# ogulcanaydogan/llm-slo-ebpf-toolkit

Measured on AMD Instinct MI355X. Metric: fault-replay attribution throughput through the agent's BPF-ring -> GPU path (events/s, node-wide); held-out attribution macro-F1 and agent CPU overhead % reported alongside, higher is better.
Workload: dtype fp64 posteriors / fp32 features (exact-int64 time joins)

## Files before the change

### llm_slo_ebpf_toolkit_amd/ops/csrc/agent_bindings.cpp

```cpp
#include <pybind11/numpy.h>
#include <pybind11/pybind11.h>
#include <pybind11/stl.h>

#include <cstring>
#include <memory>
#include <stdexcept>

#include "decodesli.h"
#include "drift.h"
#include "engine.h"
#include "errsli.h"
#include "exemplars.h"
#include "onset.h"
#include "openreq.h"
#include "podrank.h"
#include "slisketch.h"

namespace py = pybind11;
using namespace mislo;

namespace {

template <class T>
py::array_t<T> copy_array(const T* p, std::vector<py::ssize_t> shape) {
// ... 1222 lines not shown
      .def("resident", &PyErrorSliTracker::resident)
      .def("sync", &PyErrorSliTracker::sync)
      .def("close", &PyErrorSliTracker::close);
  py::class_<PyEngine>(m, "WindowEngine")
      .def(py::init<int, int, int, int, int, int, int, double, double, int, int, bool, bool, int, float, double, int,
                    int, int, int, int, bool>(),
           py::arg("device") = 0, py::arg("sig_cap") = 1 << 20, py::arg("span_cap") = 16384, py::arg("group_cap") = 64,
           py::arg("user_cap") = 1 << 18, py::arg("n_buffers") = 3, py::arg("max_ahead") = 3,
           py::arg("window_ms") = 2000.0, py::arg("threshold") = 0.7, py::arg("fanout") = 3, py::arg("group_mode") = 1,
           py::arg("use_graphs") = true, py::arg("device_refit") = true, py::arg("n_dom") = 10,
           py::arg("ttft_slo_ms") = 800.0f, py::arg("halo_ms") = 0.0, py::arg("import_cap") = 0,
           py::arg("xchg_cap") = 0, py::arg("shard_rank") = 0, py::arg("shard_world") = 1,
           py::arg("halo_windows") = 3, py::arg("split_rings") = false)
      .def("register_host", &PyEngine::register_host)
      .def("submit", &PyEngine::submit, py::arg("k"), py::arg("kernel"), py::arg("user"), py::arg("spans"),
           py::arg("n_groups"), py::arg("labels") = py::none(), py::arg("bases") = std::vector<int64_t>{},
           py::arg("with_labels") = true, py::arg("learn") = false, py::arg("user_rec") = 64)
      .def("submit_copy", &PyEngine::submit_copy, py::arg("k"), py::arg("kernel"), py::arg("user"), py::arg("spans"),
           py::arg("n_groups"), py::arg("labels") = py::none(), py::arg("bases") = std::vector<int64_t>{},
           py::arg("user_rec") = 64)
      .def("submit_chain", &PyEngine::submit_chain, py::arg("k"), py::arg("n_groups"), py::arg("with_labels") = true,
           py::arg("learn") = false)
      .def("h2d_done", &PyEngine::h2d_done)
      .def("wait_h2d", &PyEngine::wait_h2d)
      .def("query", &PyEngine::query)
      .def("wait", &PyEngine::wait)
      .def("packet", &PyEngine::packet)
      .def("results", &PyEngine::results)
      .def("window_ms", &PyEngine::window_ms)
      .def("copy_ms", [](PyEngine& p, int64_t k) {
        py::gil_scoped_release nogil;
        return p.eng().copy_ms(k);
      })
      .def("set_model_bytes", &PyEngine::set_model_bytes)
      .def("set_app_model", &PyEngine::set_app_model)
      .def("set_p0", &PyEngine::set_p0)
      .def("set_refit", &PyEngine::set_refit, py::arg("alpha") = 2.0, py::arg("prior_pseudo") = 1.0,
           py::arg("inv_temp") = 1.0, py::arg("min_count") = 0.0, py::arg("cap_dom") = -1, py::arg("ceil") = 1.0)
      .def("refit_now", &PyEngine::refit_now)
      .def("set_device_refit", [](PyEngine& p, bool on) { p.eng().set_device_refit(on); })
      .def("score", &PyEngine::score, py::arg("feat"), py::arg("labels") = py::none(), py::arg("app") = py::none())
      .def("set_pods", &PyEngine::set_pods)
      .def("inject_remote", &PyEngine::inject_remote)
      .def("results_all", &PyEngine::results_all)
      .def("set_join_params", &PyEngine::set_join_params)
      .def("init_comm", &PyEngine::init_comm)
      .def("totals", &PyEngine::totals)
      .def("reset_totals", &PyEngine::reset_totals)
      .def("stats_acc", &PyEngine::stats_acc)
      .def("model_bytes", &PyEngine::model_bytes)
      .def("restore", &PyEngine::restore)
      .def("sync", &PyEngine::sync)
      .def("import_state", &PyEngine::import_state)
      .def("sent_block", &PyEngine::sent_block)
      .def("close", &PyEngine::close)
      .def_property_readonly("buffers", &PyEngine::buffers)
      .def_property_readonly("copy_lanes", [](PyEngine& p) { return p.eng().copy_lanes(); })
      .def_property_readonly("copy_ahead", [](PyEngine& p) { return p.eng().copy_ahead(); })
      .def("take_copy_lanes", [](PyEngine& p) {
        py::gil_scoped_release nogil;
        return p.eng().take_copy_lanes();
      })
      .def_property_readonly("windows_folded", &PyEngine::folded)
      .def_property_readonly("graphs", &PyEngine::graphs)
      .def_property_readonly("host_issue_us", &PyEngine::host_issue_us)
      .def_property_readonly("host_wait_us", &PyEngine::host_wait_us)
// ... 12 lines not shown
```

### llm_slo_ebpf_toolkit_amd/ops/csrc/decode.hip

```cpp
#include "mislo_common.h"
#include "mislo_launch.h"
#include <stdexcept>

namespace mislo {

__constant__ Tables c_tab;

struct DecodeOut {
  SignalCols cols;
  uint32_t* hist;
  uint32_t* status_cnt;
  uint32_t* part_cnt;
  unsigned long long* misc;
  int blk_base = 0;
  uint32_t* sel_cnt = nullptr;
  unsigned long long* sel_mask = nullptr;
  int sel_stride = 0;
};

constexpr int kMiscSums = 2;

template <int NT>
__device__ __forceinline__ void store_counts(const uint32_t* lds, uint32_t* dst) {
  for (int i = threadIdx.x; i < kKeyTypes * kParts; i += NT) dst[i] = lds[i];
}

struct DecodeLds {
  alignas(16) Tables tab;
  static constexpr int kRep = 8, kPartRep = 4;
  static constexpr int kHS = kSlots * kBuckets + 1, kSS = kSlots * 3 + 1, kUS = kSlots + 1;
  static constexpr int kPS = kKeyTypes * kParts + 1;
  uint32_t hist[kRep * kHS];
  uint32_t status[kRep * kSS];
  uint32_t part[kPartRep * kPS];
  unsigned long long sum[kRep * kUS];
};

template <int NT>
__device__ __forceinline__ void lds_init(DecodeLds& L) {
  static_assert(sizeof(Tables) % 4 == 0 && offsetof(Tables, edges) % 16 == 0, "table layout");
  {
    const uint32_t* src = reinterpret_cast<const uint32_t*>(&c_tab);
    uint32_t* dst = reinterpret_cast<uint32_t*>(&L.tab);
    for (int i = threadIdx.x; i < (int)(sizeof(Tables) / 4); i += NT) dst[i] = src[i];
  }
  for (int i = threadIdx.x; i < DecodeLds::kPartRep * DecodeLds::kPS; i += NT) L.part[i] = 0;
  for (int i = threadIdx.x; i < DecodeLds::kRep * DecodeLds::kUS; i += NT) L.sum[i] = 0;
  for (int i = threadIdx.x; i < DecodeLds::kRep * DecodeLds::kHS; i += NT) L.hist[i] = 0;
  for (int i = threadIdx.x; i < DecodeLds::kRep * DecodeLds::kSS; i += NT) L.status[i] = 0;
  __syncthreads();
}

struct LdsLane {
  uint32_t *hist, *status, *part;
  unsigned long long* sum;
  const Tables* tab;
};
__device__ __forceinline__ LdsLane lds_lane(DecodeLds& L) {
  const int r = threadIdx.x & (DecodeLds::kRep - 1), q = threadIdx.x & (DecodeLds::kPartRep - 1);
  return LdsLane{L.hist + r * DecodeLds::kHS, L.status + r * DecodeLds::kSS, L.part + q * DecodeLds::kPS,
                 L.sum + r * DecodeLds::kUS, &L.tab};
}
// ... 585 lines not shown
    }
    PartCodes pc;
#pragma unroll
    for (int k = 0; k < kKeyTypes; ++k) {
      const uint64_t h = r.ts != 0 ? key_hash(k, r.tr, r.pod, r.pid, r.cn, r.sn) : 0ull;
      pc.p[k] = h ? (uint16_t)part_of(h) : kNoPart;
      if (h) atomicAdd(&s_part[k * kParts + part_of(h)], 1u);
    }
    c.part[i] = pc;
  }
  if (sm.gen) {
    for (int off = 32; off > 0; off >>= 1) {
      t_lo = min(t_lo, (uint64_t)__shfl_xor((long long)t_lo, off));
      t_hi = max(t_hi, (uint64_t)__shfl_xor((long long)t_hi, off));
    }
    if ((threadIdx.x & 63) == 0 && t_lo <= t_hi) {
      atomicMin(reinterpret_cast<unsigned long long*>(&sm.gen->span_lo), (unsigned long long)t_lo);
      atomicMax(reinterpret_cast<unsigned long long*>(&sm.gen->span_hi), (unsigned long long)t_hi);
    }
  }
  __syncthreads();
  store_counts<NT>(s_part, part_cnt + (size_t)blockIdx.x * kKeyTypes * kParts);
  if (sli_lds)
    for (int i = threadIdx.x; i < 2 * sm.n_groups; i += NT)
      if (s_sli[i]) atomicAdd(&sm.grp_sli[i], s_sli[i]);
  if (app_lds)
    for (int i = threadIdx.x; i < 2 * sm.n_groups; i += NT)
      if (s_app[i]) atomicAdd(&sm.grp_app[i], s_app[i]);
  if (late_lds)
    for (int i = threadIdx.x; i < sm.n_groups; i += NT)
      if (s_late[i]) atomicAdd(&sm.grp_late[2 * i], s_late[i]);
}

constexpr int kDecodeNT = 1024;

int decode_sel_stride(int cap) {
  const long long g = decode_grid(cap), chunk = ((long long)cap + g - 1) / g;
  return (int)((chunk + kDecodeNT - 1) / kDecodeNT) * (kDecodeNT / 64);
}

int decode_grid(int cap) {
  long long g = ((long long)cap + 1023) / 1024;
  if (g < 1) g = 1;
  if (g > kPartBlocks) g = kPartBlocks;
  return (int)g;
}

void set_tables(const Tables* host_tables) {
  (void)hipMemcpyToSymbol(HIP_SYMBOL(c_tab), host_tables, sizeof(Tables), 0, hipMemcpyHostToDevice);
}

void launch_decode_events(const void* ev, const int* n_dev, int cap, const SignalCols& cols, uint32_t* hist,
                          uint32_t* status_cnt, uint32_t* part_cnt, unsigned long long* misc, hipStream_t stream) {
  DecodeOut o{cols, hist, status_cnt, part_cnt, misc};
  constexpr int NT = kDecodeNT;
  hipLaunchKernelGGL((k_decode_events<NT>), dim3(decode_grid(cap)), dim3(NT), 0, stream,
                     (const Event*)ev, n_dev, cap, o);
}

void launch_decode_wire(const void* ev, const int* n_dev, int cap, const uint32_t* ctx_tab, int n_ctx,
                        const SignalCols& cols, uint32_t* hist, uint32_t* status_cnt, uint32_t* part_cnt,
                        unsigned long long* misc, hipStream_t stream) {
  DecodeOut o{cols, hist, status_cnt, part_cnt, misc};
  constexpr int NT = kDecodeNT;
  hipLaunchKernelGGL((k_decode_wire<NT, EventC16>), dim3(decode_grid(cap)), dim3(NT), 0, stream,
                     (const EventC16*)ev, n_dev, cap, reinterpret_cast<const uint4*>(ctx_tab), n_ctx, o);
}
// ... 45 lines not shown
```

### llm_slo_ebpf_toolkit_amd/ops/csrc/engine.h

```cpp
#pragma once

#include <hip/hip_runtime.h>
#include <rccl/rccl.h>

#include <map>
#include <tuple>
#include <type_traits>
#include <vector>

#include "copylanes.h"
#include "mislo_launch.h"
#include "mislo_packet.h"

namespace mislo {

constexpr uint32_t kCtxRows = 1u << 24;
constexpr uint32_t kPodRows = 1u << 20;
constexpr uint32_t kTraceIdRows = 1u << 24;
constexpr int kHeadBytes = 64;

struct Seg {
  const void* ptr;
  size_t bytes;
};
// ... 60 lines not shown
  int user_rec = 64;
  std::vector<Seg> spans;
  int n_groups = 0;
  const int32_t* labels = nullptr;
  int64_t bases[4] = {0, 0, 0, 0};
};

class WindowEngine {
 public:
  explicit WindowEngine(const EngineConfig& cfg);
  ~WindowEngine();
  WindowEngine(const WindowEngine&) = delete;
  WindowEngine& operator=(const WindowEngine&) = delete;

  const EngineConfig& config() const { return cfg_; }
  int buffers() const { return nb_; }

  bool register_host(const void* ptr, size_t bytes);
  void submit(int64_t k, const WindowInput& in, bool with_labels, bool learn);
  void submit_copy(int64_t k, const WindowInput& in);
  void submit_chain(int64_t k, int n_groups, bool with_labels, bool learn);
  bool copy_ahead() const { return copy_ahead_; }
  bool h2d_done(int64_t k);
  void wait_h2d(int64_t k);
  int copy_lanes() const { return lanes_; }
  bool take_copy_lanes();
  bool query(int64_t k);
  void wait(int64_t k);
  const double* packet(int64_t k) const { return bufs_[k % nb_].packet_host; }
  ResultView results(int64_t k) const { return layout().view<const uint8_t>(bufs_[k % nb_].res_host); }
  ResultLayout layout() const { return ResultLayout{(size_t)cfg_.group_cap}; }
  std::pair<float, float> window_ms(int64_t k);
  std::vector<float> copy_ms(int64_t k);

  void set_model_bytes(const void* bytes, size_t n);
  void set_refit(double alpha, double prior_pseudo, double inv_temp, double min_count, int cap_dom = -1,
                 double ceil = 1.0);
  void refit_now();
  void set_device_refit(bool on) { cfg_.device_refit = on; }
  void score_features(const float* feat, int n, const int32_t* labels, double* post, int32_t* pred, double* conf,
                      uint32_t* evbits, uint32_t* confusion, const uint32_t* app_cnt = nullptr);
  void set_app_model(const void* bytes, size_t n);
  void set_p0(const double* p0, size_t n);
  void set_pods(const uint32_t* pods, const uint32_t* svcnode, size_t n);
  void inject_remote(const void* blocks, size_t stride, int world, int me);
  void set_join_params(double window_ms, double threshold, int fanout, int group_mode);
  void init_comm(const ncclUniqueId& id, int rank, int world);
  bool has_comm() const { return comm_ != nullptr; }
  int rank() const { return rank_; }
  int world() const { return world_; }
  const uint8_t* results_all(int64_t k) const { return comm_ ? bufs_[k % nb_].res_all_host : bufs_[k % nb_].res_host; }
  size_t result_bytes() const { return layout().bytes(); }

  void totals(double* out);
  void reset_totals();
  void stats_acc(double* out);
  void restore(const double* stats, const void* model, size_t model_bytes, int64_t folded);
  void model_bytes(void* out);
  void sync();
  std::vector<int64_t> import_state();
  std::vector<uint8_t> sent_block();
  int64_t windows_folded() const { return folded_; }
  size_t staged_bytes() const { return staged_bytes_; }
  size_t direct_bytes() const { return direct_bytes_; }
  size_t graphs() const { return graphs_.size(); }
  double host_issue_us() const { return issue_n_ ? issue_us_ / issue_n_ : 0.0; }
// ... 64 lines not shown
  size_t inject_stride_ = 0;
  int inject_world_ = 0, inject_me_ = 0;
  int rank_ = 0, world_ = 1;
  hipStream_t side_ = nullptr;
  hipStream_t front_ = nullptr;
  bool overlap_ = false;
  struct BufSet {
    GenMeta* gen;
    int* rows;
    uint32_t *ring_state, *hist, *status, *confusion, *cnt, *gcnt;
    unsigned long long *misc, *dbg, *top3, *gsum;
    double *stats, *stats_count;
    SpanRec* s_rec;
    PartCodes* s_part;
    uint32_t *s_items, *s_part_base, *probe_work;
    PreSpan* s_pre;
  };
  std::vector<BufSet> sets_;
  struct Buf {
    int b;
    uint8_t* in;
    uint8_t* head_host;
    uint8_t* staging;
    double *packet_dev, *packet_host;
    uint8_t *res_dev, *res_host;
    uint8_t *res_all_dev, *res_all_host;
    ResultViewT<uint8_t> res;
    SigRec* imp;
    uint32_t* remote_n;
    const BufSet* set;
    const GenMeta* gen_prev;
    hipEvent_t head_done, front_done, compute_done, comm_done, xchg_done;
    hipEvent_t t_comp0, t_comp1, t_end;
    const int* counts() const { return reinterpret_cast<const int*>(in); }
  };
  std::vector<Buf> bufs_;
  struct CopyMark {
    hipEvent_t t_start, h2d_done;
  };
  std::vector<CopyMark> marks_;
  const CopyMark& mark(int64_t k) const { return marks_[copy_mark_slot(k, nb_)]; }
  hipEvent_t ev_fork_ = nullptr, ev_sigbase_ = nullptr, ev_spans_ = nullptr;
  bool branch_ = false;
  bool xspan_ = false;
  bool exchange() const { return comm_ && cfg_.xchg_cap > 0 && cfg_.import_cap > 0; }
  JoinParams jp_{};
  int nblk_sig_ = 1, nblk_span_ = 1;
  hipStream_t copy_[kMaxCopyLanes] = {nullptr, nullptr};
  int lanes_ = 1;
  bool copy_ahead_ = false;
  bool lane_on_request_ = false;
  bool copy_open_ = false;
  int copy_groups_ = 0;
  int64_t copied_windows() const { return submitted_ + (copy_open_ ? 1 : 0); }
  CopiedUpTo copied_;
  bool copied_ready(int64_t w, bool block);
  hipStream_t compute_ = nullptr, comm_stream_ = nullptr;
  ncclComm_t comm_ = nullptr;
  ncclComm_t xcomm_ = nullptr;
  uint32_t* ctx_tab_ = nullptr;
  double *totals_ = nullptr, *stats_acc_ = nullptr, *p0_ = nullptr;
  uint8_t* model_dev_ = nullptr;
  std::vector<uint8_t*> model_host_;
  int model_slot_ = 0;
  uint8_t* g_status_ = nullptr;
  PartCodes* g_part_ = nullptr;
  uint32_t *g_part_blk_ = nullptr, *g_part_off_ = nullptr, *g_part_tot_ = nullptr, *g_part_base_ = nullptr,
           *g_items_ = nullptr;
  SigRec* g_rec_ = nullptr;
// ... 24 lines not shown
```

### llm_slo_ebpf_toolkit_amd/ops/csrc/engine.hip

```cpp
#include "engine.h"
#include "mislo_packet_kernels.h"

#include <algorithm>
#include <chrono>
#include <cstdlib>
#include <cmath>
#include <cstring>
#include <stdexcept>
#include <string>

namespace mislo {

namespace {

#define HIPCHECK(x)                                                                                  \
  do {                                                                                               \
    hipError_t _e = (x);                                                                             \
    if (_e != hipSuccess) throw std::runtime_error(std::string("HIP error: ") + hipGetErrorString(_e) + \
                                                   " at " #x);                                       \
  } while (0)

#define NCCLCHECK(x)                                                                                        \
  do {                                                                                                      \
    ncclResult_t _r = (x);                                                                                  \
    if (_r != ncclSuccess) throw std::runtime_error(std::string("RCCL error: ") + ncclGetErrorString(_r) + \
                                                    " at " #x);                                             \
  } while (0)

__global__ void k_accumulate(const double* __restrict__ packet, double* __restrict__ totals, int n,
                             double* __restrict__ host) {
  const int i = blockIdx.x * blockDim.x + threadIdx.x;
  if (i < n) {
    const double v = packet[i];
    totals[i] += v;
    host[i] = v;
  }
}

__global__ __launch_bounds__(256) void k_window_end(const uint32_t* hist, const uint32_t* status,
                                                    const unsigned long long* misc, const unsigned long long* dbg,
// ... 119 lines not shown
}

void WindowEngine::set_join_params(double window_ms, double threshold, int fanout, int group_mode) {
  const int64_t ms = 1000000;
  int64_t outer = (int64_t)llround(window_ms * ms);
  if (outer <= 0) outer = 2000 * ms;
  if (outer >= (1LL << 35)) throw std::invalid_argument("window too large for top-3 key packing (< 34 s)");
  jp_.outer_ns = outer;
  const int64_t tw[4] = {outer, 100 * ms, 250 * ms, 500 * ms};
  for (int k = 0; k < 4; ++k) jp_.win_ns[k] = std::min(outer, tw[k]);
  const float cf[4] = {1.0f, 0.9f, 0.8f, 0.65f};
  for (int k = 0; k < 4; ++k) jp_.conf[k] = cf[k];
  jp_.threshold = threshold > 0 ? (float)threshold : 0.7f;
  if (fanout <= 0) fanout = 3;
  if (fanout > 3) throw std::invalid_argument("GPU join keeps at most 3 candidates per span");
  jp_.fanout = fanout;
  jp_.group_mode = group_mode;
  graphs_.clear();
}

void WindowEngine::alloc() {
  const int64_t S = cfg_.span_cap, G = cfg_.group_cap;
  n_rows_ = cfg_.sig_cap + cfg_.import_cap;
  const int64_t N = n_rows_;
  nblk_sig_ = decode_grid((int)N);
  nblk_span_ = decode_grid((int)S);
  const bool one_stream = env_int("MISLO_ONE_STREAM", 0) == 1;
  compute_ = mk_stream();
  copy_[0] = one_stream ? compute_ : mk_stream();
  spin_ = env_int("MISLO_SPIN_WAIT", 0) == 1;
  overlap_ = env_int("MISLO_WINDOW_OVERLAP", !one_stream) == 1 && !one_stream &&
             !(cfg_.xchg_cap > 0 && cfg_.import_cap > 0);
  if (overlap_) front_ = mk_stream();
  copy_ahead_ = overlap_ && env_int("MISLO_COPY_AHEAD", kCopyAheadDefault) == 1;
  const char* lanes_env = getenv("MISLO_COPY_LANES");
  lanes_ = overlap_ && (lanes_env ? atoi(lanes_env) == 2 : nb_ >= 4) ? 2 : 1;
  lane_on_request_ = copy_ahead_ && !lanes_env && lanes_ == 1 && nb_ >= 3;
  copy_[1] = lanes_ == 2 ? mk_stream(env_int("MISLO_COPY_LANE_PRIO", 1) != 0) : copy_[0];
  slots_ = gens_ + (overlap_ ? 1 : 0);
  {
    if (env_int("MISLO_SPAN_STREAM", !one_stream && !overlap_) == 1) enable_span_branch();
  }
  comm_stream_ = compute_;
  const size_t head = (kHeadBytes + 4 * (size_t)G + 63) & ~size_t(63);
  off_kern_ = head;
  off_user_ = (off_kern_ + kern_bytes() + 63) & ~size_t(63);
  off_span_ = off_user_ + 64 * (size_t)cfg_.user_cap;
  in_bytes_ = off_span_ + 64 * (size_t)S;
  const ResultLayout lay = layout();
  bufs_.assign(nb_, Buf{});
  for (Buf& buf : bufs_) {
    buf.in = dalloc<uint8_t>(in_bytes_, true);
    buf.head_host = static_cast<uint8_t*>(host_block(head));
    buf.packet_dev = dalloc<double>(kPacketLen, true);
    buf.packet_host = static_cast<double*>(host_block(kPacketLen * sizeof(double)));
    for (hipEvent_t* e : {&buf.head_done, &buf.compute_done, &buf.comm_done, &buf.front_done, &buf.xchg_done})
      *e = mk_event(kEvWait);
    for (hipEvent_t* e : {&buf.t_comp0, &buf.t_comp1, &buf.t_end}) *e = mk_event(hipEventDefault);
    buf.res_host = static_cast<uint8_t*>(host_block(lay.bytes()));
    buf.res_dev = dalloc<uint8_t>(lay.bytes(), true);
    buf.res = lay.view(buf.res_dev);
    buf.imp = cfg_.import_cap ? dalloc<SigRec>(cfg_.import_cap) : nullptr;
  }
  marks_.assign((size_t)copy_mark_slots(nb_), CopyMark{});
  for (CopyMark& m : marks_) {
    m.t_start = mk_event(hipEventDefault);
    m.h2d_done = mk_event(hipEventBlockingSync);
  }
  warm_.assign(kStageSlots * nb_, false);
  pod_sn_ = dalloc<uint32_t>(kPodRows, true);
  pod_host_ = static_cast<uint32_t*>(host_alloc(kPodRows * 4, hipHostMallocDefault));
  std::memset(pod_host_, 0, kPodRows * 4);
  trace_hash_ = dalloc<unsigned long long>(kTraceIdRows, true);
  tmax_ = dalloc<unsigned long long>(1, true);
  remote_n_ = dalloc<uint32_t>(nb_, true);
  for (int i = 0; i < (overlap_ ? nb_ : 1); ++i) {
    BufSet s{};
    s.rows = dalloc<int>(16, true);
    s.ring_state = dalloc<uint32_t>(kRsLen);
    s.gen = dalloc<GenMeta>(1);
    GenMeta g{};
    g.cur = (uint32_t)slots_ - 1;
    for (int a = 0; a < kMaxGens; ++a) g.cut[a] = INT64_MAX;
    HIPCHECK(hipMemcpy(s.gen, &g, sizeof(g), hipMemcpyHostToDevice));
    s.s_part = dalloc<PartCodes>(S);
    s.s_part_base = dalloc<uint32_t>(kKeyTypes * kParts + 1);
    s.s_items = dalloc<uint32_t>(kKeyTypes * S);
    s.s_pre = dalloc<PreSpan>((size_t)kKeyTypes * S);
    s.s_rec = dalloc<SpanRec>(S);
    s.probe_work = dalloc<uint32_t>(kProbeWorkLen, true);
    s.top3 = dalloc<unsigned long long>(3 * S);
// ... 224 lines not shown
    launch_posterior(r.feat, counts + 2, G, pm, with_labels ? labels : nullptr, r.post, r.pred, r.gconf, r.evbits,
                     s.confusion, st, app_dev_, r.app);
  if (!comm_) {
    const size_t res16 = (result_bytes() + 15) / 16;
    const int g = (int)std::max<size_t>((kPacketLen + 255) / 256, std::min<size_t>(64, (res16 + 255) / 256));
    hipLaunchKernelGGL(k_window_end, dim3(g), dim3(256), 0, st, s.hist, s.status, s.misc, s.dbg, s.confusion, s.stats,
                       s.stats_count, s.ring_state, buf.packet_dev, totals_, buf.packet_host,
                       reinterpret_cast<const uint4*>(buf.res_dev), reinterpret_cast<uint4*>(buf.res_host), res16);
    return;
  }
  hipLaunchKernelGGL(k_pack, dim3((kPacketLen + 255) / 256), dim3(256), 0, st, s.hist, s.status, s.misc, s.dbg,
                     s.confusion, s.stats, s.stats_count, s.ring_state, buf.packet_dev);
}

void WindowEngine::run_spans(const Buf& buf, hipStream_t st) {
  const BufSet& s = *buf.set;
  const int* counts = buf.counts();
  const int S = cfg_.span_cap, G = cfg_.group_cap;
  const SpanMap sm{1, buf.res.sli, G, cfg_.ttft_slo_ms, cfg_.shard_rank, cfg_.shard_world,
                   s.gen, buf.res.app, buf.res.late};
  launch_decode_spans(buf.in + off_span_, counts + 1, S, span_cols(buf), s_part_blk_, ctx_tab_, (int)kCtxRows, st, &sm);
  launch_partition(s.s_part, counts + 1, S, nblk_span_, s_part_blk_, s_part_off_, s_part_tot_, s.s_part_base, s.s_items,
                   st);
  launch_span_sort(span_cols(buf), s.s_items, s.s_part_base, s.s_pre, st);
}

void WindowEngine::run_span_branch(const Buf& buf, hipStream_t st) {
  HIPCHECK(hipEventRecord(ev_fork_, st));
  HIPCHECK(hipStreamWaitEvent(side_, ev_fork_, 0));
  run_spans(buf, side_);
}

void WindowEngine::launch_part(Stage part, const Buf& buf, int n_groups, bool with_labels, bool learn) {
  hipStream_t cs = part == Stage::XchgSpans ? side_ : part == Stage::Front ? front_ : compute_;
  auto run = [&] {
    switch (part) {
      case Stage::Window:
        run_part1(buf, cs, false);
        run_join_front(buf, cs, false);
        return run_join_back(buf, n_groups, with_labels, learn, cs);
      case Stage::Records: return run_part1(buf, cs, true);
      case Stage::Join:
        run_join_front(buf, cs, true);
        return run_join_back(buf, n_groups, with_labels, learn, cs);
      case Stage::XchgSpans: return run_spans(buf, cs);
      case Stage::XchgHead: return run_begin(buf, cs);
      case Stage::Front:
        run_part1(buf, cs, false);
        return run_join_front(buf, cs, false);
      case Stage::Back: return run_join_back(buf, n_groups, with_labels, learn, cs);
    }
  };
  if (!cfg_.use_graphs) return run();
  const int slot = buf.b * kStageSlots + (int)part;
  auto key = part == Stage::Front ? std::make_tuple(slot, 0, false, false)
                                  : std::make_tuple(slot, n_groups, with_labels, learn);
  auto it = graphs_.find(key);
  if (it == graphs_.end() && !warm_[slot]) {
    run();
    warm_[slot] = true;
    return;
  }
  if (it == graphs_.end()) {
    hipGraph_t g;
    HIPCHECK(hipStreamBeginCapture(cs, hipStreamCaptureModeThreadLocal));
    run();
    HIPCHECK(hipStreamEndCapture(cs, &g));
// ... 99 lines not shown
  Lap part;
  dma(in.kernel, buf.in + off_kern_, kern_bytes(), buf.staging, st_off, cs);
  part(split_us_[0]);
  part(split_us_[1]);
  dma(in.user, buf.in + off_user_, 64 * (size_t)cfg_.user_cap, buf.staging, st_off, cs);
  part(split_us_[2]);
  dma(in.spans, buf.in + off_span_, 64 * (size_t)cfg_.span_cap, buf.staging, st_off, cs);
  part(split_us_[3]);
  HIPCHECK(hipEventRecord(mk.h2d_done, cs));
  phase(dma_us_);
  copy_open_ = true;
  copy_groups_ = n_groups;
  whole(issue_us_);
}

void WindowEngine::submit_chain(int64_t k, int n_groups, bool with_labels, bool learn) {
  Lap whole;
  if (!copy_open_ || k != submitted_) throw std::logic_error("submit_chain: not the window submit_copy queued last");
  if (n_groups != copy_groups_) throw std::invalid_argument("submit_chain: n_groups differs from the copy phase's");
  Buf& buf = bufs_[k % nb_];
  const CopyMark& mk = mark(k);
  Lap phase;
  if (copy_ahead_ && k >= max_ahead_) HIPCHECK(hipEventSynchronize(bufs_[(k - max_ahead_) % nb_].compute_done));
  phase(wait_us_);
  hipStream_t fs = overlap_ ? front_ : compute_;
  HIPCHECK(hipStreamWaitEvent(fs, mk.h2d_done, 0));
  if (overlap_ && k >= 2) HIPCHECK(hipStreamWaitEvent(fs, bufs_[(k - 2) % nb_].compute_done, 0));
  HIPCHECK(hipStreamWaitEvent(compute_, buf.comm_done, 0));
  const bool injected = !inject_.empty();
  if (injected) {
    HIPCHECK(hipMemcpyAsync(xrecv_, inject_.data(), inject_.size(), hipMemcpyHostToDevice, compute_));
    HIPCHECK(hipStreamSynchronize(compute_));
  }
  HIPCHECK(hipEventRecord(buf.t_comp0, fs));
  to_host(buf.head_host, buf.in, off_kern_, fs);
  HIPCHECK(hipEventRecord(buf.head_done, fs));
  if (cfg_.device_refit && k >= nb_) {
    refit(buf.packet_dev + kStatsOff);
    ++folded_;
  }
  const bool xchg = exchange() || injected;
  phase(pre_us_);
  if (overlap_) {
    if (xchg) throw std::logic_error("the exchange path does not run with overlapped windows");
    launch_part(Stage::Front, buf, n_groups, with_labels, learn);
    HIPCHECK(hipEventRecord(buf.front_done, front_));
    HIPCHECK(hipStreamWaitEvent(compute_, buf.front_done, 0));
    launch_part(Stage::Back, buf, n_groups, with_labels, learn);
  } else if (!xchg) {
    launch_part(Stage::Window, buf, n_groups, with_labels, learn);
  } else {
    if (xspan_) {
      launch_part(Stage::XchgHead, buf, n_groups, with_labels, learn);
      HIPCHECK(hipEventRecord(ev_fork_, compute_));
      HIPCHECK(hipStreamWaitEvent(side_, ev_fork_, 0));
      launch_part(Stage::XchgSpans, buf, n_groups, with_labels, learn);
      HIPCHECK(hipEventRecord(ev_spans_, side_));
    }
    launch_part(Stage::Records, buf, n_groups, with_labels, learn);
    if (injected) {
      merge_remote(buf, xrecv_, inject_stride_, inject_world_, inject_me_, compute_);
      inject_.clear();
    } else if (xcomm_) {
      NCCLCHECK(ncclAllGather(xsend_, xrecv_, xstride_, ncclUint8, xcomm_, compute_));
      merge_remote(buf, xrecv_, xstride_, world_, rank_, compute_);
    } else {
      HIPCHECK(hipEventRecord(buf.xchg_done, compute_));
      HIPCHECK(hipStreamWaitEvent(comm_stream_, buf.xchg_done, 0));
      NCCLCHECK(ncclAllGather(xsend_, xrecv_, xstride_, ncclUint8, comm_, comm_stream_));
      merge_remote(buf, xrecv_, xstride_, world_, rank_, comm_stream_);
      HIPCHECK(hipEventRecord(buf.xchg_done, comm_stream_));
      HIPCHECK(hipStreamWaitEvent(compute_, buf.xchg_done, 0));
    }
    if (xspan_) HIPCHECK(hipStreamWaitEvent(compute_, ev_spans_, 0));
    launch_part(Stage::Join, buf, n_groups, with_labels, learn);
  }
  phase(launch_us_);
  const size_t res_bytes = result_bytes();
  if (comm_) to_host(buf.res_dev, buf.res_host, res_bytes, compute_);
  HIPCHECK(hipEventRecord(buf.t_comp1, compute_));
// ... 23 lines not shown
  if (e == hipSuccess) return true;
  if (e == hipErrorNotReady) return false;
  HIPCHECK(e);
  return false;
}

void WindowEngine::wait(int64_t k) {
  if (spin_) {
    while (!query(k)) {
    }
    return;
  }
  HIPCHECK(hipEventSynchronize(bufs_[k % nb_].comm_done));
}

std::vector<float> WindowEngine::copy_ms(int64_t k) {
  const CopyMark& mk = mark(k);
  float dur = 0.f, gap = -1.f;
  HIPCHECK(hipEventSynchronize(mk.h2d_done));
  HIPCHECK(hipEventElapsedTime(&dur, mk.t_start, mk.h2d_done));
  if (k >= 1) HIPCHECK(hipEventElapsedTime(&gap, mark(k - 1).h2d_done, mk.t_start));
  return {dur, gap};
}

std::pair<float, float> WindowEngine::window_ms(int64_t k) {
  const Buf& buf = bufs_[k % nb_];
  float total = 0.f, comp = 0.f;
  HIPCHECK(hipEventSynchronize(buf.t_end));
  HIPCHECK(hipEventElapsedTime(&total, mark(k).t_start, buf.t_end));
  HIPCHECK(hipEventElapsedTime(&comp, buf.t_comp0, buf.t_comp1));
  return {total, comp};
}

void WindowEngine::set_model_bytes(const void* bytes, size_t n) {
  if (n != sizeof(PosteriorModel)) throw std::invalid_argument("model image must be POSTERIOR_MODEL_BYTES bytes");
  uint8_t* h = model_host_[model_slot_++ % model_host_.size()];
  std::memcpy(h, bytes, n);
  HIPCHECK(hipMemcpyAsync(model_dev_, h, n, hipMemcpyHostToDevice, compute_));
}

void WindowEngine::set_app_model(const void* bytes, size_t n) {
  if (n != sizeof(AppModel)) throw std::invalid_argument("application model must be APP_MODEL_BYTES bytes");
  uint8_t* h = model_host_[model_slot_++ % model_host_.size()];
  static_assert(sizeof(AppModel) <= sizeof(PosteriorModel), "the staging slots fit the application model");
  std::memcpy(h, bytes, n);
  HIPCHECK(hipMemcpyAsync(app_dev_, h, n, hipMemcpyHostToDevice, compute_));
}

void WindowEngine::set_p0(const double* p0, size_t n) {
  if (n != (size_t)kSlots * 16 && n != 2 * (size_t)kSlots * 16) throw std::invalid_argument("p0 must be f64[256] or [512]");
  HIPCHECK(hipMemset(p0_ + kSlots * 16, 0, kSlots * 16 * sizeof(double)));
  HIPCHECK(hipMemcpy(p0_, p0, n * sizeof(double), hipMemcpyHostToDevice));
}

void WindowEngine::set_refit(double alpha, double prior_pseudo, double inv_temp, double min_count, int cap_dom,
                             double ceil) {
  if (!(alpha > 0.0) || !(prior_pseudo >= 0.0) || !(inv_temp > 0.0) || !(min_count >= 0.0) || cap_dom >= cfg_.n_dom ||
      !(ceil > 0.0 && ceil <= 1.0))
    throw std::invalid_argument("refit parameters");
  cfg_.lik_ceil = ceil;
  cfg_.cap_dom = cap_dom < 0 ? -1 : cap_dom;
  cfg_.alpha = alpha;
  cfg_.prior_pseudo = prior_pseudo;
  cfg_.inv_temp = inv_temp;
  cfg_.min_count = min_count;
}
// ... 59 lines not shown
  for (int a = 0; a < kMaxGens; ++a) out.push_back(g.cut[a]);
  for (int a = 0; a < kMaxGens; ++a) out.push_back(a < gens_ ? g.n_rows[(g.cur + slots_ - a) % slots_] : 0);
  for (int b = 0; b < nb_; ++b) out.push_back(r[b]);
  return out;
}

void WindowEngine::inject_remote(const void* blocks, size_t stride, int world, int me) {
  if (!cfg_.import_cap || !cfg_.xchg_cap) throw std::logic_error("inject_remote needs import_cap and xchg_cap > 0");
  if (world < 1 || me < 0 || me >= world || stride < sizeof(XRec)) throw std::invalid_argument("bad exchange blocks");
  const uint8_t* h = static_cast<const uint8_t*>(blocks);
  for (int r = 0; r < world; ++r) {
    uint32_t c;
    std::memcpy(&c, h + (size_t)r * stride, 4);
    if ((size_t)c * sizeof(XRec) + sizeof(XRec) > stride) throw std::invalid_argument("block row count exceeds stride");
    if (r != me && c > (uint32_t)cfg_.xchg_cap) throw std::invalid_argument("block holds more rows than xchg_cap");
  }
  if (stride * world > xrecv_bytes_) {
    sync();
    own_.free_dev(xrecv_);
    xrecv_ = dalloc<uint8_t>(stride * world);
    xrecv_bytes_ = stride * world;
  }
  inject_.assign(h, h + stride * world);
  inject_stride_ = stride;
  inject_world_ = world;
  inject_me_ = me;
}

void WindowEngine::init_comm(const ncclUniqueId& id, int rank, int world) {
  if (comm_) throw std::logic_error("communicator already initialised");
  if (world < 1 || rank < 0 || rank >= world) throw std::invalid_argument("communicator rank / world");
  if (submitted_ || copy_open_) throw std::logic_error("init_comm before the first window");
  HIPCHECK(hipSetDevice(cfg_.device));
  if (overlap_) {
    HIPCHECK(hipStreamSynchronize(front_));
    overlap_ = false;
    copy_ahead_ = lane_on_request_ = false;
    lanes_ = 1;
    if (!getenv("MISLO_SPAN_STREAM")) enable_span_branch();
  }
  NCCLCHECK(ncclCommInitRank(&comm_, world, id, rank));
  {
    comm_stream_ = mk_stream(env_int("MISLO_COMM_STREAM_PRIO", 1) != 0);
  }
  rank_ = rank;
  world_ = world;
  for (Buf& buf : bufs_) {
    buf.res_all_dev = dalloc<uint8_t>(result_bytes() * world);
    buf.res_all_host = static_cast<uint8_t*>(host_block(result_bytes() * world));
  }
  if (cfg_.xchg_cap) {
    if (world > 8) throw std::invalid_argument("the exchange is sized for <= 8 GPUs per node");
    own_.free_dev(xrecv_);
    xrecv_bytes_ = xstride_ * world;
    xrecv_ = dalloc<uint8_t>(xrecv_bytes_, true);
    const char* xv = getenv("MISLO_XCHG_STREAM");
    int split = (xv && std::strcmp(xv, "compute") == 0) ? 1 : 0;
    int* d_split = dalloc<int>(1);
    HIPCHECK(hipMemcpy(d_split, &split, sizeof(int), hipMemcpyHostToDevice));
    NCCLCHECK(ncclBroadcast(d_split, d_split, 1, ncclInt32, 0, comm_, comm_stream_));
    HIPCHECK(hipStreamSynchronize(comm_stream_));
    HIPCHECK(hipMemcpy(&split, d_split, sizeof(int), hipMemcpyDeviceToHost));
    own_.free_dev(d_split);
    if (split) NCCLCHECK(ncclCommSplit(comm_, 0, rank, &xcomm_, nullptr));
  }
}
// ... 44 lines not shown
```

### llm_slo_ebpf_toolkit_amd/ops/csrc/exchange.hip

```cpp
#include "mislo_common.h"
#include "mislo_launch.h"
#include "mislo_packet.h"

namespace mislo {

namespace {

constexpr int kSelNT = 256;

struct SelArgs {
  SignalCols gc;
  const int* rows;
  const int* counts;
  int cap;
};

__device__ __forceinline__ int sel_end(const SelArgs& a) { return min(a.counts[0], min(a.rows[0], a.cap)); }

__device__ __forceinline__ const SigRec* sel_rows(const SelArgs& a) {
  return a.gc.rec + (size_t)cur_slot(a.gc) * (size_t)a.gc.stride;
}

__device__ __forceinline__ bool selected(const SelArgs& a, const SigRec& r, int i) {
  if (r.slot == kNoSlot || r.ts == 0) return false;
// ... 201 lines not shown
  }
  if (blockIdx.x == 0 && threadIdx.x == 0) {
    if (gen) gen_begin_body(gen, gen_prev ? gen_prev : gen, *tmax, gens, slots, halo_ns);
    *tmax = 0ull;
    ring_state[kRsFirstBusy] = 0xFFFFFFFFu;
    for (int j = 1; j < kRsLen; ++j) ring_state[j] = 0u;
    *remote_n = 0u;
    window_rows_body(counts, 0u, cap, rows, gen);
  }
}

}

int select_grid(int cap) {
  int g = (cap + 4095) / 4096;
  return g < 1 ? 1 : (g > 1024 ? 1024 : g);
}

void launch_select(const SignalCols& gc, const int* rows, const int* counts, int cap, uint32_t* blk_cnt,
                   uint32_t* blk_off, XRec* out, uint32_t* n_out, uint32_t out_cap, hipStream_t stream,
                   unsigned long long* dropped) {
  const SelArgs a{gc, rows, counts, cap};
  const int g = select_grid(cap);
  hipLaunchKernelGGL(k_sel_count, dim3(g), dim3(kSelNT), 0, stream, a, blk_cnt);
  hipLaunchKernelGGL(k_sel_scan, dim3(1), dim3(1024), 0, stream, blk_cnt, g, blk_off, n_out, out_cap, dropped);
  hipLaunchKernelGGL(k_sel_scatter, dim3(g), dim3(kSelNT), 0, stream, a, blk_off, out, out_cap);
}

void launch_select_masked(const SignalCols& gc, const int* rows, int cap, const uint32_t* blk_cnt, uint32_t* blk_off,
                          const unsigned long long* mask, int mask_stride, XRec* out, uint32_t* n_out,
                          uint32_t out_cap, hipStream_t stream, unsigned long long* dropped) {
  const int g = decode_grid(cap);
  hipLaunchKernelGGL(k_sel_scan, dim3(1), dim3(1024), 0, stream, blk_cnt, g, blk_off, n_out, out_cap, dropped);
  hipLaunchKernelGGL((k_sel_scatter_mask<1024>), dim3(g), dim3(1024), 0, stream, gc, rows, cap, mask, mask_stride,
                     blk_off, out, out_cap);
}

void launch_remote_merge(const uint8_t* xrecv, size_t stride, int world, int me, SigRec* imp, uint32_t* remote_n,
                         uint32_t imp_cap, int max_rows, hipStream_t stream, unsigned long long* dropped) {
  int g = (max_rows + 255) / 256;
  g = g < 1 ? 1 : (g > 1024 ? 1024 : g);
  hipLaunchKernelGGL(k_remote_merge, dim3(g), dim3(256), 0, stream, xrecv, stride, world, me, imp, remote_n, imp_cap,
                     dropped);
}

void launch_window_rows(const int* counts, const uint32_t* remote_n, int cap, int* rows, GenMeta* gen,
                        hipStream_t stream) {
  hipLaunchKernelGGL(k_window_rows, dim3(1), dim3(64), 0, stream, counts, remote_n, cap, rows, gen);
}

void launch_window_begin(const FillList& fl, GenMeta* gen, const GenMeta* gen_prev, unsigned long long* tmax, int gens,
                         int slots, long long halo_ns, uint32_t* ring_state, uint32_t* remote_n, const int* counts,
                         int cap, int* rows, hipStream_t stream) {
  hipLaunchKernelGGL(k_window_begin, dim3(256), dim3(256), 0, stream, fl, gen, gen_prev, tmax, gens, slots, halo_ns,
                     ring_state, remote_n, counts, cap, rows);
}

}
```

### llm_slo_ebpf_toolkit_amd/ops/csrc/join.hip

```cpp
#include <cstdlib>

#include "mislo_common.h"
#include "mislo_launch.h"

namespace mislo {

constexpr int kSigBits = 27;
constexpr int kChunk = 256;


constexpr int kScanCols = 32, kScanRG = 32;
__global__ __launch_bounds__(kScanCols * kScanRG) void k_part_scan(const uint32_t* __restrict__ part_blk, int nblk,
                                                                  uint32_t* __restrict__ part_off,
                                                                  uint32_t* __restrict__ part_tot) {
  __shared__ uint32_t s_sum[kScanRG][kScanCols];
  const int cl = threadIdx.x % kScanCols, r = threadIdx.x / kScanCols;
  const int c = blockIdx.x * kScanCols + cl;
  const int per = (nblk + kScanRG - 1) / kScanRG;
  const int b0 = min(nblk, r * per), b1 = min(nblk, b0 + per);
  constexpr size_t W = (size_t)kKeyTypes * kParts;
  uint32_t sum = 0;
  for (int b = b0; b < b1; ++b) sum += part_blk[(size_t)b * W + c];
  s_sum[r][cl] = sum;
  __syncthreads();
// ... 277 lines not shown
  if (p == 0) {
    uint32_t run = 0;
    for (int q = 0; q < 64; ++q) {
      const uint32_t v = s_cls[q];
      s_cls[q] = run;
      run += v;
    }
  }
  __syncthreads();
#pragma unroll
  for (int k = 1; k < kKeyTypes; ++k)
#pragma unroll
    for (int a = 0; a < kMaxGens; ++a)
      for (uint32_t j = 0; j < n[k][a]; ++j) {
        const uint32_t pos = atomicAdd(&s_cls[63u - probe_item_class(k, slice(k, a, j), ns[k])], 1u);
        items2[pos] = code(k, a, j);
      }
  if (p == 0) {
    work[0] = t[0];
    work[1] = t[1] + t[2] + t[3];
    work[2] = 0u;
    work[3] = 0u;
  }
}

__global__ __launch_bounds__(kParts) void k_probe_work(const uint32_t* __restrict__ span_base, SignalCols gc,
                                                       JoinParams jp, int sig_per_item, uint32_t* __restrict__ work) {
  __shared__ unsigned long long s[kParts], s2[kParts];
  __shared__ uint32_t s_cls[64];
  probe_work_body(span_base, gc, jp, sig_per_item, work, s, s2, s_cls);
}

template <int NT>
__global__ __launch_bounds__(NT) void k_scatter_sig_work(SignalCols gc, const int* __restrict__ n_ptr, int cap,
                                                         const uint32_t* __restrict__ part_off, int nblk_a,
                                                         const uint32_t* __restrict__ span_base, JoinParams jp,
                                                         int sig_per_item, uint32_t* __restrict__ work) {
  static_assert(NT == kParts, "the work-list block runs one thread per partition");
  static_assert(2 * kParts * 8 + 64 * 4 >= kKeyTypes * kParts * 4, "one LDS buffer serves both");
  __shared__ unsigned long long s_buf[2 * kParts + 32];
  if (blockIdx.x == 0) {
    probe_work_body(span_base, gc, jp, sig_per_item, work, s_buf, s_buf + kParts,
                    reinterpret_cast<uint32_t*>(s_buf + 2 * kParts));
    return;
  }
  scatter_sig_body<NT>(gc, n_ptr, cap, part_off, nblk_a, (int)blockIdx.x - 1, (int)gridDim.x - 1,
                       reinterpret_cast<uint32_t*>(s_buf));
}

template <int NT>
__device__ __forceinline__ void block_inclusive_scan(int* v, int n, int* wsum) {
  const int t = threadIdx.x, lane = t & 63, wave = t >> 6;
  const int i0 = 2 * t, i1 = 2 * t + 1;
  const int a = i0 < n ? v[i0] : 0, b = i1 < n ? v[i1] : 0;
  const int local = a + b;
  int incl = local;
  for (int off = 1; off < 64; off <<= 1) {
    const int y = __shfl_up(incl, off);
    if (lane >= off) incl += y;
  }
  if (lane == 63) wsum[wave] = incl;
  __syncthreads();
  int base = 0;
  for (int w = 0; w < wave; ++w) base += wsum[w];
  const int excl = base + incl - local;
  if (i0 < n) v[i0] = excl + a;
  if (i1 < n) v[i1] = excl + a + b;
// ... 114 lines not shown
    if (ti < m) {
      const uint32_t rid = (uint32_t)(s_aux[i] - 1);
      store_prespan(out + c0 + i, s_kt[i].h, s_kt[i].t, rr, my_s, rid | (s_ok[rid] << 16));
    }
  }
}

template <int NT, bool LG>
__global__ __launch_bounds__(NT, LG ? 4 : 6) void k_probe(const PreSpan* __restrict__ pre,
                                              const uint32_t* __restrict__ span_base, SignalCols gc, int span_cap,
                                              JoinParams jp, unsigned long long* __restrict__ top3,
                                              uint32_t* __restrict__ cnt, int n_groups,
                                              unsigned long long* __restrict__ gsum, uint32_t* __restrict__ gcnt,
                                              unsigned long long* __restrict__ dbg, uint32_t* __restrict__ work,
                                              int phase) {
  static_assert(kChunk == NT, "staging keeps one span per thread");
  __shared__ SpanKT s_kt[kChunk];
  __shared__ SpanTC s_tc[kChunk];
  __shared__ SpanPP s_pp[kChunk];
  __shared__ uint32_t s_i[kChunk];
  __shared__ unsigned long long s_top[kChunk * 3];
  __shared__ unsigned long long s_seed3[kChunk];
  __shared__ int s_diff[kChunk + 1];
  __shared__ int s_aux[kChunk];
  __shared__ uint16_t s_rid[kChunk];
  __shared__ uint32_t s_runok[kChunk];
  __shared__ uint16_t s_needy[kChunk];
  __shared__ int s_wsum[NT / 64];
  __shared__ int s_nneedy;
  __shared__ uint32_t s_item;
  constexpr int kLg = LG ? kLdsGroups * kSlots : 1;
  __shared__ unsigned long long s_gsum[kLg];
  __shared__ uint32_t s_gcnt[kLg];

  {
    const size_t stripe = (size_t)(blockIdx.x & (kGroupStripes - 1)) * (size_t)n_groups * kSlots;
    gsum += stripe;
    gcnt += stripe;
  }
  const bool grp_lds = LG && n_groups <= kLdsGroups;
  const bool any_groups = jp.group_mode == 1 && n_groups > 0;
  if (grp_lds && any_groups) {
    for (int i = threadIdx.x; i < kLdsGroups * kSlots; i += NT) {
      s_gsum[i] = 0ull;
      s_gcnt[i] = 0u;
    }
  }
  const bool cand1 = jp.conf[1] >= jp.threshold, cand2 = jp.conf[2] >= jp.threshold;
  unsigned long long n_cand = 0, n_low = 0, n_overlap = 0;
  const uint32_t n_work = work[phase];
  const uint32_t* items = work + 4 + (phase ? kProbePhaseItems : 0);
  const uint32_t cur = cur_slot(gc);

  for (;;) {
    __syncthreads();
    if (threadIdx.x == 0) s_item = atomicAdd(&work[2 + phase], 1u);
    __syncthreads();
    const uint32_t it = s_item;
    if (it >= n_work) break;
#ifdef MISLO_PROBE_PROFILE
    unsigned long long pt = clock64(), p_stage = 0, p_sig = 0, p_flush = 0;
#endif
    const uint32_t code = items[it];
    const int k = (int)(code >> 30);
    const int age = (int)((code >> 28) & 3u);
    const int part = (int)((code >> 16) & 0x3FF);
// ... 537 lines not shown
```

### llm_slo_ebpf_toolkit_amd/ops/csrc/mislo_common.h

```cpp
#pragma once

#include <hip/hip_runtime.h>
#include <stdint.h>

namespace mislo {

constexpr int kSlots = 16;
constexpr int kBuckets = 16;
constexpr int kKeyTypes = 4;
#ifndef MISLO_PART_BITS
#define MISLO_PART_BITS 10
#endif
constexpr int kPartBits = MISLO_PART_BITS;
constexpr int kParts = 1 << kPartBits;
static_assert(kPartBits >= 6 && kPartBits <= 10, "partition table sizes assume 64..1024 partitions");
constexpr int kPartBlocks = 256;
constexpr int kMaxDomains = 16;
constexpr int kMaxPairs = 48;
constexpr int kGroupStripes = 16;
constexpr int kMaxTypes = 128;
constexpr uint64_t kEmpty = ~0ull;
constexpr uint8_t kNoSlot = 0xFF;

struct alignas(64) Event {
  int64_t ts_ns;
  uint64_t value;
  uint64_t trace_h;
  uint32_t pid, tid, pod_id, dst_ip;
  uint16_t signal_type, node_id, svc_id, flags, src_port, dst_port;
  int32_t err;
  uint64_t conn_h;
};
static_assert(sizeof(Event) == 64, "Event must be 64 bytes");

struct alignas(32) User32 {
  int64_t ts_ns;
  uint64_t trace_h;
  uint32_t value_milli, pod_id, pid;
  uint8_t signal_type, flags;
  uint16_t node_id;
};
static_assert(sizeof(User32) == 32, "User32 must be 32 bytes");

struct alignas(8) User24 {
  uint64_t trace_h;
  uint32_t value_milli;
  uint32_t ts_lo;
  uint32_t pid_sig;
  uint32_t pod_ts;
// ... 206 lines not shown
```

### llm_slo_ebpf_toolkit_amd/ops/csrc/mislo_launch.h

```cpp
#pragma once

#include <hip/hip_runtime.h>
#include <stdint.h>

#include "mislo_common.h"
#include "mislo_packet.h"

namespace mislo {

struct PosteriorModel {
  double w[kSlots][kMaxDomains];
  double bias[kMaxDomains];
  double mean[kSlots];
  double nominal[kSlots];
  float thr[kSlots];
  uint32_t dom_mask[kMaxDomains];
  uint32_t table_mask;
  int32_t mode;
  int32_t n_pairs;
  double pair_rho;
  double w2[kSlots][kMaxPairs];
  double bias2[kMaxPairs];
  uint8_t pair_a[kMaxPairs];
  uint8_t pair_b[kMaxPairs];
};

constexpr int kAppBit = 16;
struct AppModel {
  double w[kMaxDomains];
  double b[kMaxDomains];
  double w2[kMaxPairs];
  double b2[kMaxPairs];
  double thr_ms;
  uint32_t dom_mask;
  int32_t on;
};

void set_tables(const Tables* host_tables);
int decode_grid(int cap);
void launch_decode_events(const void* ev, const int* n_dev, int cap, const SignalCols& cols, uint32_t* hist,
                          uint32_t* status_cnt, uint32_t* part_cnt, unsigned long long* misc, hipStream_t stream);
void launch_decode_wire(const void* ev, const int* n_dev, int cap, const uint32_t* ctx_tab, int n_ctx,
                        const SignalCols& cols, uint32_t* hist, uint32_t* status_cnt, uint32_t* part_cnt,
                        unsigned long long* misc, hipStream_t stream);
void launch_decode_ref(const void* ev, const int* n_dev, int cap, uint32_t pod, uint32_t svcnode, uint64_t trace_h,
                       const SignalCols& cols, uint32_t* hist, uint32_t* status_cnt, uint32_t* part_cnt,
                       unsigned long long* misc, hipStream_t stream);
struct SpanMap {
  int native;
  uint32_t* grp_sli;
  int n_groups;
  float ttft_slo_ms;
  int sh_rank = 0, sh_world = 1;
  GenMeta* gen = nullptr;
  uint32_t* grp_app = nullptr;
  uint32_t* grp_late = nullptr;
};
constexpr double kAppUnitsPerMs = 100.0;
void launch_decode_spans(const void* sp, const int* n_dev, int cap, const SpanCols& cols, uint32_t* part_cnt,
                         const uint32_t* ctx_tab, int n_ctx, hipStream_t stream, const SpanMap* sm = nullptr);
void launch_ring_defs(const uint8_t* framed, const int* n_dev, int cap, uint32_t* ctx_tab, uint32_t ctx_rows,
                      const uint32_t* pod_sn, uint32_t n_pods, const TraceIds& tt, uint32_t* ring_state,
                      hipStream_t stream);
void launch_decode_window(const uint8_t* framed, const void* user, const int* n_dev, const int* rows, int cap,
                          const SigRec* imp, const uint32_t* ctx_tab, int n_ctx, const TraceIds& tt,
                          uint32_t* ring_state, unsigned long long* tmax, const uint32_t* pod_sn, uint32_t n_pods,
                          const SignalCols& cols, uint32_t* hist, uint32_t* status_cnt, uint32_t* part_cnt,
                          unsigned long long* misc, hipStream_t stream, int seg = 0, int grid = 0, int blk_base = 0,
                          int sh_rank = 0, int sh_world = 1, uint32_t* sel_cnt = nullptr,
                          unsigned long long* sel_mask = nullptr, int sel_stride = 0);
int decode_sel_stride(int cap);
// ... 84 lines not shown
```

Measured before the change: 2.661 billion.

## Shrink decode workgroup and LDS so front decode co-resides with probe workgroups

Cuts the decode kernel block size from 1024 to 512 threads and halves the partition-count LDS replicas. The aim is for the front-stage decode to fit on a CU next to two probe workgroups, so the overlapped front and back streams can actually run concurrently. It also adds a launch_bounds occupancy hint to the signal scatter kernel, static_asserts that guard the LDS budget, and optional per-stage event timing behind MISLO_STAGE_TIMES. In exchange, each decode block has fewer threads and fewer LDS replicas, so contention on shared atomics within a block may rise.

```diff
diff --git a/llm_slo_ebpf_toolkit_amd/ops/csrc/agent_bindings.cpp b/llm_slo_ebpf_toolkit_amd/ops/csrc/agent_bindings.cpp
--- a/llm_slo_ebpf_toolkit_amd/ops/csrc/agent_bindings.cpp
+++ b/llm_slo_ebpf_toolkit_amd/ops/csrc/agent_bindings.cpp
@@ -1278,6 +1278,21 @@
         py::gil_scoped_release nogil;
         return p.eng().copy_ms(k);
       })
+      .def_property_readonly("stage_times", [](PyEngine& p) { return p.eng().stage_times(); })
+      .def("stage_ms", [](PyEngine& p, int64_t k) {
+        std::vector<float> t;
+        {
+          py::gil_scoped_release nogil;
+          t = p.eng().stage_ms(k);
+        }
+        py::dict d;
+        d["front_ms"] = t[0];
+        d["back_start_ms"] = t[1];
+        d["back_end_ms"] = t[2];
+        d["back_offset_ms"] = t[3];
+        d["t0_ms"] = t[4];
+        return d;
+      })
       .def("set_model_bytes", &PyEngine::set_model_bytes)
       .def("set_app_model", &PyEngine::set_app_model)
       .def("set_p0", &PyEngine::set_p0)
diff --git a/llm_slo_ebpf_toolkit_amd/ops/csrc/decode.hip b/llm_slo_ebpf_toolkit_amd/ops/csrc/decode.hip
--- a/llm_slo_ebpf_toolkit_amd/ops/csrc/decode.hip
+++ b/llm_slo_ebpf_toolkit_amd/ops/csrc/decode.hip
@@ -27,7 +27,7 @@
 
 struct DecodeLds {
   alignas(16) Tables tab;
-  static constexpr int kRep = 8, kPartRep = 4;
+  static constexpr int kRep = 8, kPartRep = 2;
   static constexpr int kHS = kSlots * kBuckets + 1, kSS = kSlots * 3 + 1, kUS = kSlots + 1;
   static constexpr int kPS = kKeyTypes * kParts + 1;
   uint32_t hist[kRep * kHS];
@@ -679,7 +679,9 @@
       if (s_late[i]) atomicAdd(&sm.grp_late[2 * i], s_late[i]);
 }
 
-constexpr int kDecodeNT = 1024;
+static_assert(kDecodeNT % 64 == 0 && kDecodeNT >= kSlots, "whole waves; lds_flush sums one slot per thread");
+static_assert(lds_alloc(sizeof(DecodeLds) + kDecodeNT * 5 * sizeof(uint4) + 64) <= kFrontLdsBudget,
+              "k_decode_window no longer fits on a CU beside two probe workgroups");
 
 int decode_sel_stride(int cap) {
   const long long g = decode_grid(cap), chunk = ((long long)cap + g - 1) / g;
diff --git a/llm_slo_ebpf_toolkit_amd/ops/csrc/engine.h b/llm_slo_ebpf_toolkit_amd/ops/csrc/engine.h
--- a/llm_slo_ebpf_toolkit_amd/ops/csrc/engine.h
+++ b/llm_slo_ebpf_toolkit_amd/ops/csrc/engine.h
@@ -116,6 +116,8 @@
   ResultLayout layout() const { return ResultLayout{(size_t)cfg_.group_cap}; }
   std::pair<float, float> window_ms(int64_t k);
   std::vector<float> copy_ms(int64_t k);
+  bool stage_times() const { return stage_times_; }
+  std::vector<float> stage_ms(int64_t k);
 
   void set_model_bytes(const void* bytes, size_t n);
   void set_refit(double alpha, double prior_pseudo, double inv_temp, double min_count, int cap_dom = -1,
@@ -246,9 +248,18 @@
     const GenMeta* gen_prev;
     hipEvent_t head_done, front_done, compute_done, comm_done, xchg_done;
     hipEvent_t t_comp0, t_comp1, t_end;
+    hipEvent_t t_front1 = nullptr, t_back0 = nullptr;
+    int64_t staged_k = -1;
     const int* counts() const { return reinterpret_cast<const int*>(in); }
   };
   std::vector<Buf> bufs_;
+  struct StageMarks {
+    float front0, front1, back0, back1;
+  };
+  bool stage_times_ = false;
+  hipEvent_t stage_base_ = nullptr;
+  std::vector<StageMarks> stage_log_;
+  void read_stage_marks(int64_t k);
   struct CopyMark {
     hipEvent_t t_start, h2d_done;
   };
diff --git a/llm_slo_ebpf_toolkit_amd/ops/csrc/engine.hip b/llm_slo_ebpf_toolkit_amd/ops/csrc/engine.hip
--- a/llm_slo_ebpf_toolkit_amd/ops/csrc/engine.hip
+++ b/llm_slo_ebpf_toolkit_amd/ops/csrc/engine.hip
@@ -6,6 +6,7 @@
 #include <cstdlib>
 #include <cmath>
 #include <cstring>
+#include <limits>
 #include <stdexcept>
 #include <string>
 
@@ -191,6 +192,7 @@
   overlap_ = env_int("MISLO_WINDOW_OVERLAP", !one_stream) == 1 && !one_stream &&
              !(cfg_.xchg_cap > 0 && cfg_.import_cap > 0);
   if (overlap_) front_ = mk_stream();
+  stage_times_ = env_int("MISLO_STAGE_TIMES", 0) == 1 && !(cfg_.xchg_cap > 0 && cfg_.import_cap > 0);
   copy_ahead_ = overlap_ && env_int("MISLO_COPY_AHEAD", kCopyAheadDefault) == 1;
   const char* lanes_env = getenv("MISLO_COPY_LANES");
   lanes_ = overlap_ && (lanes_env ? atoi(lanes_env) == 2 : nb_ >= 4) ? 2 : 1;
@@ -216,6 +218,8 @@
     for (hipEvent_t* e : {&buf.head_done, &buf.compute_done, &buf.comm_done, &buf.front_done, &buf.xchg_done})
       *e = mk_event(kEvWait);
     for (hipEvent_t* e : {&buf.t_comp0, &buf.t_comp1, &buf.t_end}) *e = mk_event(hipEventDefault);
+    if (stage_times_)
+      for (hipEvent_t* e : {&buf.t_front1, &buf.t_back0}) *e = mk_event(hipEventDefault);
     buf.res_host = static_cast<uint8_t*>(host_block(lay.bytes()));
     buf.res_dev = dalloc<uint8_t>(lay.bytes(), true);
     buf.res = lay.view(buf.res_dev);
@@ -506,7 +510,7 @@
 }
 
 void WindowEngine::launch_part(Stage part, const Buf& buf, int n_groups, bool with_labels, bool learn) {
-  hipStream_t cs = part == Stage::XchgSpans ? side_ : part == Stage::Front ? front_ : compute_;
+  hipStream_t cs = part == Stage::XchgSpans ? side_ : part == Stage::Front && overlap_ ? front_ : compute_;
   auto run = [&] {
     switch (part) {
       case Stage::Window:
@@ -672,6 +676,15 @@
     HIPCHECK(hipMemcpyAsync(xrecv_, inject_.data(), inject_.size(), hipMemcpyHostToDevice, compute_));
     HIPCHECK(hipStreamSynchronize(compute_));
   }
+  const bool staged = stage_times_ && !injected && !exchange();
+  if (stage_times_) {
+    if (k >= nb_) read_stage_marks(k - nb_);
+    if (!stage_base_) {
+      stage_base_ = mk_event(hipEventDefault);
+      HIPCHECK(hipEventRecord(stage_base_, fs));
+    }
+    buf.staged_k = staged ? k : -1;
+  }
   HIPCHECK(hipEventRecord(buf.t_comp0, fs));
   to_host(buf.head_host, buf.in, off_kern_, fs);
   HIPCHECK(hipEventRecord(buf.head_done, fs));
@@ -685,7 +698,14 @@
     if (xchg) throw std::logic_error("the exchange path does not run with overlapped windows");
     launch_part(Stage::Front, buf, n_groups, with_labels, learn);
     HIPCHECK(hipEventRecord(buf.front_done, front_));
+    if (staged) HIPCHECK(hipEventRecord(buf.t_front1, front_));
     HIPCHECK(hipStreamWaitEvent(compute_, buf.front_done, 0));
+    if (staged) HIPCHECK(hipEventRecord(buf.t_back0, compute_));
+    launch_part(Stage::Back, buf, n_groups, with_labels, learn);
+  } else if (staged) {
+    launch_part(Stage::Front, buf, n_groups, with_labels, learn);
+    HIPCHECK(hipEventRecord(buf.t_front1, compute_));
+    HIPCHECK(hipEventRecord(buf.t_back0, compute_));
     launch_part(Stage::Back, buf, n_groups, with_labels, learn);
   } else if (!xchg) {
     launch_part(Stage::Window, buf, n_groups, with_labels, learn);
@@ -775,6 +795,29 @@
   return {total, comp};
 }
 
+void WindowEngine::read_stage_marks(int64_t k) {
+  if ((int64_t)stage_log_.size() > k) return;
+  const float nan = std::numeric_limits<float>::quiet_NaN();
+  stage_log_.resize((size_t)k + 1, StageMarks{nan, nan, nan, nan});
+  const Buf& buf = bufs_[k % nb_];
+  if (buf.staged_k != k) return;
+  StageMarks& m = stage_log_[(size_t)k];
+  HIPCHECK(hipEventSynchronize(buf.t_comp1));
+  HIPCHECK(hipEventElapsedTime(&m.front0, stage_base_, buf.t_comp0));
+  HIPCHECK(hipEventElapsedTime(&m.front1, stage_base_, buf.t_front1));
+  HIPCHECK(hipEventElapsedTime(&m.back0, stage_base_, buf.t_back0));
+  HIPCHECK(hipEventElapsedTime(&m.back1, stage_base_, buf.t_comp1));
+}
+
+std::vector<float> WindowEngine::stage_ms(int64_t k) {
+  if (!stage_times_) throw std::logic_error("stage_ms: the engine was not built with MISLO_STAGE_TIMES=1");
+  if (k < 0 || k >= submitted_) throw std::invalid_argument("stage_ms: the window has not been submitted");
+  for (int64_t w = std::max<int64_t>((int64_t)stage_log_.size(), submitted_ - nb_); w <= k; ++w) read_stage_marks(w);
+  const StageMarks& m = stage_log_[(size_t)k];
+  const float off = k >= 1 ? m.back0 - stage_log_[(size_t)k - 1].back1 : std::numeric_limits<float>::quiet_NaN();
+  return {m.front1 - m.front0, m.back0 - m.front0, m.back1 - m.front0, off, m.front0};
+}
+
 void WindowEngine::set_model_bytes(const void* bytes, size_t n) {
   if (n != sizeof(PosteriorModel)) throw std::invalid_argument("model image must be POSTERIOR_MODEL_BYTES bytes");
   uint8_t* h = model_host_[model_slot_++ % model_host_.size()];
@@ -900,6 +943,7 @@
   if (world < 1 || rank < 0 || rank >= world) throw std::invalid_argument("communicator rank / world");
   if (submitted_ || copy_open_) throw std::logic_error("init_comm before the first window");
   HIPCHECK(hipSetDevice(cfg_.device));
+  stage_times_ = false;
   if (overlap_) {
     HIPCHECK(hipStreamSynchronize(front_));
     overlap_ = false;
diff --git a/llm_slo_ebpf_toolkit_amd/ops/csrc/exchange.hip b/llm_slo_ebpf_toolkit_amd/ops/csrc/exchange.hip
--- a/llm_slo_ebpf_toolkit_amd/ops/csrc/exchange.hip
+++ b/llm_slo_ebpf_toolkit_amd/ops/csrc/exchange.hip
@@ -257,8 +257,8 @@
                           uint32_t out_cap, hipStream_t stream, unsigned long long* dropped) {
   const int g = decode_grid(cap);
   hipLaunchKernelGGL(k_sel_scan, dim3(1), dim3(1024), 0, stream, blk_cnt, g, blk_off, n_out, out_cap, dropped);
-  hipLaunchKernelGGL((k_sel_scatter_mask<1024>), dim3(g), dim3(1024), 0, stream, gc, rows, cap, mask, mask_stride,
-                     blk_off, out, out_cap);
+  hipLaunchKernelGGL((k_sel_scatter_mask<kDecodeNT>), dim3(g), dim3(kDecodeNT), 0, stream, gc, rows, cap, mask,
+                     mask_stride, blk_off, out, out_cap);
 }
 
 void launch_remote_merge(const uint8_t* xrecv, size_t stride, int world, int me, SigRec* imp, uint32_t* remote_n,
diff --git a/llm_slo_ebpf_toolkit_amd/ops/csrc/join.hip b/llm_slo_ebpf_toolkit_amd/ops/csrc/join.hip
--- a/llm_slo_ebpf_toolkit_amd/ops/csrc/join.hip
+++ b/llm_slo_ebpf_toolkit_amd/ops/csrc/join.hip
@@ -333,7 +333,7 @@
 }
 
 template <int NT>
-__global__ __launch_bounds__(NT) void k_scatter_sig_work(SignalCols gc, const int* __restrict__ n_ptr, int cap,
+__global__ __launch_bounds__(NT, 8) void k_scatter_sig_work(SignalCols gc, const int* __restrict__ n_ptr, int cap,
                                                          const uint32_t* __restrict__ part_off, int nblk_a,
                                                          const uint32_t* __restrict__ span_base, JoinParams jp,
                                                          int sig_per_item, uint32_t* __restrict__ work) {
@@ -514,6 +514,10 @@
   constexpr int kLg = LG ? kLdsGroups * kSlots : 1;
   __shared__ unsigned long long s_gsum[kLg];
   __shared__ uint32_t s_gcnt[kLg];
+  static_assert(sizeof(s_kt) + sizeof(s_tc) + sizeof(s_pp) + sizeof(s_i) + sizeof(s_top) + sizeof(s_seed3) +
+                        sizeof(s_diff) + sizeof(s_aux) + sizeof(s_rid) + sizeof(s_runok) + sizeof(s_needy) +
+                        sizeof(s_wsum) + sizeof(s_nneedy) + sizeof(s_item) + sizeof(s_gsum) + sizeof(s_gcnt) <= kProbeLdsBytes,
+                "the probe's LDS grew: kProbeLdsBytes and the front stage's budget follow");
 
   {
     const size_t stripe = (size_t)(blockIdx.x & (kGroupStripes - 1)) * (size_t)n_groups * kSlots;
diff --git a/llm_slo_ebpf_toolkit_amd/ops/csrc/mislo_common.h b/llm_slo_ebpf_toolkit_amd/ops/csrc/mislo_common.h
--- a/llm_slo_ebpf_toolkit_amd/ops/csrc/mislo_common.h
+++ b/llm_slo_ebpf_toolkit_amd/ops/csrc/mislo_common.h
@@ -15,6 +15,11 @@
 constexpr int kParts = 1 << kPartBits;
 static_assert(kPartBits >= 6 && kPartBits <= 10, "partition table sizes assume 64..1024 partitions");
 constexpr int kPartBlocks = 256;
+constexpr int kCuLdsBytes = 160 * 1024, kLdsGranule = 1280;
+constexpr int lds_alloc(size_t bytes) { return (int)((bytes + kLdsGranule - 1) / kLdsGranule) * kLdsGranule; }
+constexpr int kProbeResident = 2;
+constexpr int kProbeLdsBytes = 37920;
+constexpr int kFrontLdsBudget = kCuLdsBytes - kProbeResident * lds_alloc(kProbeLdsBytes);
 constexpr int kMaxDomains = 16;
 constexpr int kMaxPairs = 48;
 constexpr int kGroupStripes = 16;
diff --git a/llm_slo_ebpf_toolkit_amd/ops/csrc/mislo_launch.h b/llm_slo_ebpf_toolkit_amd/ops/csrc/mislo_launch.h
--- a/llm_slo_ebpf_toolkit_amd/ops/csrc/mislo_launch.h
+++ b/llm_slo_ebpf_toolkit_amd/ops/csrc/mislo_launch.h
@@ -37,6 +37,7 @@
 };
 
 void set_tables(const Tables* host_tables);
+constexpr int kDecodeNT = 512;
 int decode_grid(int cap);
 void launch_decode_events(const void* ev, const int* n_dev, int cap, const SignalCols& cols, uint32_t* hist,
                           uint32_t* status_cnt, uint32_t* part_cnt, unsigned long long* misc, hipStream_t stream);
```

After: 2.647 billion. About the same (-0.5%).
